# 3ickey/ConsensusML

Hardware: AMD Instinct MI355X
Metric: samples/sec ResNet-50 + Krum at 1/2/4/8 MI355X; agg overhead vs all-reduce (higher is better)
Workload: dtype bf16

## Files before the change

csrc/bindings.cpp:

```cpp
#include <torch/extension.h>
#include <array>
#include <climits>
#include <ATen/hip/HIPContext.h>
#include <c10/core/DeviceGuard.h>

#include "kernels/kernels.h"

namespace {

using at::Tensor;
using c10::optional;

#define CML_CHECK_HIP(expr)                                                               \
  do {                                                                                    \
    hipError_t _e = (expr);                                                               \
    TORCH_CHECK(_e == hipSuccess, "consensusml_amd HIP error: ", hipGetErrorString(_e), " at " \
                #expr " (bindings.cpp:", __LINE__, ")");                                  \
  } while (0)

hipStream_t cur_stream() { return c10::hip::getCurrentHIPStream().stream(); }

int dtype_of(const Tensor& t) {
  if (t.scalar_type() == at::kBFloat16) return cml::DT_BF16;
  TORCH_CHECK(t.scalar_type() == at::kFloat, "expected bf16 or fp32 tensor, got ", t.scalar_type());
// ... 1433 lines not shown
                                            cur_stream()));
  return y;
}

Tensor subsample2(const Tensor& x) {
  check_nhwc(x, "x");
  TORCH_CHECK(x.dim() == 4 && x.size(1) % 8 == 0, "subsample2: 4-D NHWC, C % 8 == 0");
  const int64_t N = x.size(0), C = x.size(1), H = x.size(2), W = x.size(3);
  const c10::DeviceGuard guard(x.device());
  Tensor y = at::empty({N, C, (H + 1) / 2, (W + 1) / 2},
                       x.options().memory_format(at::MemoryFormat::ChannelsLast));
  CML_CHECK_HIP(cml::launch_subsample2(x.data_ptr(), y.data_ptr(), static_cast<int>(N),
                                       static_cast<int>(H), static_cast<int>(W),
                                       static_cast<int>(C), cur_stream()));
  return y;
}

Tensor upsample2_scatter(const Tensor& g_in, int64_t H, int64_t W) {
  Tensor g = g_in.contiguous(at::MemoryFormat::ChannelsLast);
  check_nhwc(g, "g");
  const int64_t N = g.size(0), C = g.size(1);
  TORCH_CHECK(g.dim() == 4 && C % 8 == 0 && g.size(2) == (H + 1) / 2 && g.size(3) == (W + 1) / 2,
              "upsample2_scatter: g [N, C, ceil(H/2), ceil(W/2)], C % 8 == 0");
  const c10::DeviceGuard guard(g.device());
  Tensor dx = at::empty({N, C, H, W}, g.options().memory_format(at::MemoryFormat::ChannelsLast));
  CML_CHECK_HIP(cml::launch_upsample2_scatter(g.data_ptr(), dx.data_ptr(), static_cast<int>(N),
                                              static_cast<int>(H), static_cast<int>(W),
                                              static_cast<int>(C), cur_stream()));
  return dx;
}


Tensor wgrad3x3(const Tensor& dy_in, const Tensor& x, at::ScalarType dtype,
                const optional<Tensor>& zero_in) {
  check_nhwc(x, "x");
  Tensor dy = dy_in.contiguous(at::MemoryFormat::ChannelsLast);
  check_nhwc(dy, "dy");
  TORCH_CHECK(x.dim() == 4 && dy.dim() == 4 && dy.size(0) == x.size(0) && dy.size(2) == x.size(2) &&
                  dy.size(3) == x.size(3), "wgrad3x3: dy / x shapes");
  TORCH_CHECK(dtype == at::kBFloat16 || dtype == at::kFloat, "wgrad3x3: bf16 or fp32 output");
  const int64_t N = x.size(0), Ci = x.size(1), H = x.size(2), W = x.size(3), Co = dy.size(1);
  const c10::DeviceGuard guard(x.device());
  int S = 1, T = 0;
  TORCH_CHECK(cml::wgrad3x3_direct_plan(static_cast<int>(N), static_cast<int>(H),
                                        static_cast<int>(W), static_cast<int>(Co),
                                        static_cast<int>(Ci), &S, &T),
              "wgrad3x3: no plan for this shape (check wgrad3x3_direct_ok first)");
  Tensor zero;
  if (zero_in.has_value() && zero_in->defined()) {
    zero = *zero_in;
    TORCH_CHECK(zero.is_cuda() && zero.device() == x.device() && zero.scalar_type() == at::kBFloat16 &&
                    zero.is_contiguous() && zero.numel() >= 8, "wgrad3x3: zero must be >= 8 bf16");
  } else {
    zero = at::zeros({64}, x.options());
  }
  Tensor part = at::empty({S, Co, 9, Ci}, x.options().dtype(at::kFloat));
  Tensor dw = at::empty({Co, 3, 3, Ci}, x.options().dtype(dtype));
  CML_CHECK_HIP(cml::launch_wgrad3x3_direct(dy.data_ptr(), x.data_ptr(), zero.data_ptr(),
                                            part.data_ptr<float>(), dw.data_ptr(),
                                            dtype == at::kBFloat16, static_cast<int>(N),
                                            static_cast<int>(H), static_cast<int>(W),
                                            static_cast<int>(Co), static_cast<int>(Ci),
                                            cur_stream()));
  return dw.permute({0, 3, 1, 2});
}

bool wgrad3x3s2_ok(int64_t N, int64_t H, int64_t W, int64_t Co, int64_t Ci, int64_t taps) {
  int S = 0;
  return N < (1 << 30) && H < (1 << 15) && W < (1 << 15) && Co < (1 << 20) && Ci < (1 << 20) &&
         (taps == 9 || taps == 1) &&
         cml::wgrad3x3s2_plan(static_cast<int>(N), static_cast<int>(H), static_cast<int>(W),
                              static_cast<int>(Co), static_cast<int>(Ci), &S, static_cast<int>(taps));
}

Tensor wgrad3x3s2(const Tensor& dy_in, const Tensor& x, at::ScalarType dtype,
                  const optional<Tensor>& zero_in, int64_t taps) {
  check_nhwc(x, "x");
  Tensor dy = dy_in.contiguous(at::MemoryFormat::ChannelsLast);
  check_nhwc(dy, "dy");
  TORCH_CHECK(x.dim() == 4 && dy.dim() == 4 && dy.size(0) == x.size(0) &&
                  x.size(2) % 2 == 0 && x.size(3) % 2 == 0 && dy.size(2) * 2 == x.size(2) &&
                  dy.size(3) * 2 == x.size(3), "wgrad3x3s2: dy [N, Co, H/2, W/2], x [N, Ci, H, W]");
  TORCH_CHECK(dtype == at::kBFloat16 || dtype == at::kFloat, "wgrad3x3s2: bf16 or fp32 output");
  const int64_t N = x.size(0), Ci = x.size(1), H = x.size(2), W = x.size(3), Co = dy.size(1);
  TORCH_CHECK(wgrad3x3s2_ok(N, H, W, Co, Ci, taps),
              "wgrad3x3s2: no plan for this shape (check wgrad3x3s2_ok first)");
  const c10::DeviceGuard guard(x.device());
  int S = 1;
  cml::wgrad3x3s2_plan(static_cast<int>(N), static_cast<int>(H), static_cast<int>(W),
                       static_cast<int>(Co), static_cast<int>(Ci), &S, static_cast<int>(taps));
  Tensor zero;
  if (zero_in.has_value() && zero_in->defined()) {
    zero = *zero_in;
    TORCH_CHECK(zero.is_cuda() && zero.device() == x.device() && zero.scalar_type() == at::kBFloat16 &&
                    zero.is_contiguous() && zero.numel() >= 256 && zero.data_ptr() != nullptr &&
                    reinterpret_cast<uintptr_t>(zero.data_ptr()) % 16 == 0,
                "wgrad3x3s2: zero must be >= 256 contiguous 16-B aligned bf16");
// ... 1396 lines not shown
        py::arg("pairs"), py::arg("adapt"), py::arg("trust"), py::arg("wd"), py::arg("eps"),
        py::arg("q"), py::arg("stats"), py::arg("reduced") = py::none());
  m.def("lars_update", &lars_update, "SGD-momentum update with a per-tensor gradient factor",
        py::arg("g"), py::arg("scale"), py::arg("master"), py::arg("s1"), py::arg("q"),
        py::arg("starts"), py::arg("starts_host"), py::arg("pouts"), py::arg("offs"),
        py::arg("lens"), py::arg("lr"), py::arg("momentum"), py::arg("weight_decay"),
        py::arg("nesterov"), py::arg("first"), py::arg("grid_cap") = 0);
  m.def("bn_fwd", &bn_fwd, "fused NHWC BatchNorm(+res)(+ReLU) forward");
  m.def("bn_bwd", &bn_bwd, "fused NHWC BatchNorm(+res)(+ReLU) backward");
  m.def("bn_fwd2", &bn_fwd2, "relu(BN(x1) + BN(x2)) forward (downsample-block tail)");
  m.def("bn_bwd2", &bn_bwd2, "relu(BN(x1) + BN(x2)) backward");
  m.def("bn_relu_maxpool_fwd", &bn_relu_maxpool_fwd, "maxpool(relu(BN(x))) forward (stem)");
  m.def("stem_conv_fwd", &stem_conv_fwd, "ResNet stem 7x7/s2 conv + BN statistics (MFMA)");
  m.def("stem_wgrad", &stem_wgrad, "ResNet stem weight gradient through BN (MFMA, one pass)");
  m.def("maxpool_fwd", &maxpool_fwd, "NHWC bf16 max-pool forward (uint8 argmax)");
  m.def("maxpool_bwd", &maxpool_bwd, "NHWC bf16 max-pool backward (gather)");
  m.def("conv1x1_bn_fwd", &conv1x1_bn_fwd, py::arg("x"), py::arg("w"), py::arg("pro_sc"),
        py::arg("pro_bi"), py::arg("shift"), py::arg("running_mean"), py::arg("running_var"),
        py::arg("stride"), py::arg("stats"), py::arg("eps"), py::arg("momentum"),
        py::arg("gamma") = py::none(), py::arg("beta") = py::none(),
        "fused 1x1 conv forward (MFMA) + BN statistics epilogue + optional BN-ReLU prologue "
        "(+ with gamma / beta that BN's affine sc, bi from the statistics' finalize)");
  m.def("bn_stats", &bn_stats, "training BatchNorm statistics (mean, invstd) only");
  m.def("wgrad1x1", &wgrad1x1, py::arg("dy"), py::arg("x"), py::arg("dtype"),
        py::arg("pro_sc") = py::none(), py::arg("pro_bi") = py::none(),
        py::arg("dz_z") = py::none(), py::arg("dz_mask") = py::none(), py::arg("dz_a") = py::none(),
        py::arg("dz_b") = py::none(), py::arg("dz_c") = py::none(), py::arg("out") = py::none(),
        "weight gradient of a stride-1 1x1 conv (MFMA, split-K)");
  m.def("wgrad3x3s2_ok", &wgrad3x3s2_ok, py::arg("N"), py::arg("H"), py::arg("W"),
        py::arg("Co"), py::arg("Ci"), py::arg("taps") = 9);
  m.def("wgrad3x3s2", &wgrad3x3s2, py::arg("dy"), py::arg("x"), py::arg("dtype"),
        py::arg("zero") = py::none(), py::arg("taps") = 9);
  m.def("wgrad3x3", &wgrad3x3, py::arg("dy"), py::arg("x"), py::arg("dtype"),
        py::arg("zero") = py::none(),
        "weight gradient of a 3x3 stride-1 conv (MFMA, split-K, all nine taps per workgroup: "
        "wgrad3x3.hip) for shapes with wgrad3x3_direct_ok");
  m.def("conv1_bn_bwd_ok", &conv1_bn_bwd_ok, py::arg("M"), py::arg("p"), py::arg("Cin"),
        "whether conv1_bn_bwd takes the shape");
  m.def("conv1_bn_bwd", &conv1_bn_bwd, py::arg("dy"), py::arg("z"), py::arg("gamma"),
        py::arg("beta"), py::arg("mean"), py::arg("invstd"), py::arg("sdz"), py::arg("sdzx"),
        py::arg("x"), py::arg("w"), py::arg("dtype"), py::arg("link") = py::none(),
        py::arg("lmask") = py::none(), py::arg("link_s2") = false, py::arg("want_dz") = false,
        py::arg("splits") = 0,
        "conv1's data and weight gradients with bn1's backward apply formed on chip");
  m.def("conv1x1_link_s2", &conv1x1_link_s2,
        "1x1 data gradient + a stride-2 conv's compact data gradient at the even pixels");
  m.def("subsample2", &subsample2, "x[:, :, ::2, ::2] of an NHWC bf16 tensor, dense NHWC");
  m.def("upsample2_scatter", &upsample2_scatter, py::arg("g"), py::arg("H"), py::arg("W"),
        "full-resolution NHWC tensor with g at the even pixels, zeros elsewhere");
  m.def("wgrad3x3_direct_ok", [](int64_t B, int64_t H, int64_t W, int64_t Co, int64_t Ci) {
    int S, T;
    return cml::wgrad3x3_direct_plan(static_cast<int>(B), static_cast<int>(H), static_cast<int>(W),
                                     static_cast<int>(Co), static_cast<int>(Ci), &S, &T);
  }, "whether wgrad3x3 takes the nine-tap kernel for this shape");
  m.def("conv_gemm_bnsums", &conv_gemm_bnsums, py::arg("x"), py::arg("w"), py::arg("taps"),
        py::arg("zero"), py::arg("z"), py::arg("sc"), py::arg("bi"), py::arg("mean"),
        py::arg("invstd"), py::arg("dgamma_out") = py::none(), py::arg("dbeta_out") = py::none(),
        "stride-1 conv_gemm + the sums of the BN + ReLU backward its output feeds (+ optionally "
        "that BN's parameter gradients)");
  m.def("conv_gemm_s2dgrad", &conv_gemm_s2dgrad, py::arg("dy"), py::arg("wr"), py::arg("zero"),
        py::arg("z") = py::none(), py::arg("sc") = py::none(), py::arg("bi") = py::none(),
        py::arg("mean") = py::none(), py::arg("invstd") = py::none(),
        py::arg("dgamma_out") = py::none(), py::arg("dbeta_out") = py::none(),
        "stride-2 3x3 data gradient as four parity-class implicit GEMMs (+ BN + ReLU backward sums, "
        "+ optionally that BN's parameter gradients)");
  m.def("conv_gemm", &conv_gemm, py::arg("x"), py::arg("w"), py::arg("taps"),
        py::arg("zero") = py::none(), py::arg("stride") = 1,
        "implicit-GEMM NHWC conv (1x1 / 3x3 padding 1, stride 1 or 2), glds staging");
  m.def("conv1x1_bn_stats_only", &conv1x1_bn_stats_only, py::arg("x"), py::arg("w"),
// ... 175 lines not shown
```

csrc/kernels/kernels.h:

```cpp
#pragma once
#include <hip/hip_runtime.h>
#include <stdint.h>

namespace cml {

enum DType : int { DT_BF16 = 0, DT_F32 = 1 };
enum Combine : int { CMB_SORTED = 0, CMB_WEIGHTED = 1 };
enum Opt : int { OPT_NONE = 0, OPT_SGD = 1, OPT_ADAM = 2 };
enum Rule : int {
  RULE_MEAN = 0,
  RULE_KRUM = 1,
  RULE_MULTI_KRUM = 2,
  RULE_GEOMED = 3,
  RULE_CCLIP = 4,
  RULE_BULYAN_SELECT = 5,
  RULE_NNM_ONLY = 6,
};

struct SrcArgs {
  const void* X;
  int64_t ld;
  int n;
  int keep;
  const int* rows;
  const float* w;
  int lo, cnt;
};

struct UpdArgs {
  float* master;
  float* s1;
  float* s2;
  void* param_out;
  float* gout;
  float lr, momentum, weight_decay, beta1, beta2, eps, step_size, inv_sqrt_bc2, gscale;
// ... 253 lines not shown
bool wgrad1x1_direct(int64_t P, int Co, int Ci, bool pro = false, int dmode = 0, bool cs = false);
hipError_t launch_wgrad1x1_ex(const void* dy, const void* x, float* part, void* dw, bool dw_bf16,
                              int64_t P, int Co, int Ci, const float* pro_sc, const float* pro_bi,
                              hipStream_t st, int dmode, const void* dz_z, const uint8_t* dz_mask,
                              const float* dz_a, const float* dz_b, const float* dz_c,
                              float* cs_part, float* cs);
hipError_t launch_wgrad1x1(const void* dy, const void* x, float* part, void* dw, bool dw_bf16,
                           int64_t P, int Co, int Ci, const float* pro_sc, const float* pro_bi,
                           hipStream_t stream, const void* dz_z = nullptr,
                           const uint8_t* dz_mask = nullptr, const float* dz_a = nullptr,
                           const float* dz_b = nullptr, const float* dz_c = nullptr);

void gram1x1_plan(int64_t M, int p, int* splits, int* cps);
hipError_t launch_gram1x1(const void* z, float* part, float* G, int64_t M, int p, const float* sc,
                          const float* bi, float* cs_part, float* cy, hipStream_t st);
bool gram1x1_route(const void* dy, const void* x, int Co, int Ci, const float* pro_sc,
                   const float* pro_bi, int dmode, const float* dz_a, const float* dz_b,
                   bool dw_bf16);

bool conv1_bwd_plan(int64_t M, int p, int Cin, int* splits, int want = 0);
hipError_t launch_conv1_bwd(const void* dy, const void* z, const void* gamma, const void* beta,
                            const float* mean, const float* invstd, const float* sdz,
                            const float* sdzx, const void* x, const void* w, const void* link,
                            const uint8_t* lmask, int link_kind, int Nimg, int H, int W, void* dx,
                            float* part, int splits, void* dw, bool dw_bf16, void* dz_out,
                            int64_t M, int p, int Cin, hipStream_t st);

bool wgrad3x3s2_plan(int N, int H, int W, int Co, int Ci, int* splits, int taps = 9);
hipError_t launch_wgrad3x3s2(const void* dy, const void* x, const void* zero, float* part,
                             void* dw, bool dw_bf16, int N, int H, int W, int Co, int Ci,
                             hipStream_t st, int taps = 9);
hipError_t launch_wgrad_fold(const float* part, int S, int64_t n, void* out, bool out_bf16,
                             hipStream_t st);
bool wgrad3x3_direct_plan(int B, int H, int W, int Co, int Ci, int* splits, int* tci);
hipError_t launch_wgrad3x3_direct(const void* dy, const void* x, const void* zero, float* part,
                                  void* dw, bool dw_bf16, int B, int H, int W, int Co, int Ci,
                                  hipStream_t st);

size_t conv1x1_bn_part_floats(int64_t M, int K, int N, bool pro);
struct BnAffineOut {
  const void* gamma;
  const void* beta;
  float* sc;
  float* bi;
};
hipError_t launch_conv1x1_bn_fwd(const void* x, const void* w, void* y, float* part,
                                 const float* pro_sc, const float* pro_bi, const float* shift,
                                 int64_t M, int K, int N, int stride, int H, int W, float* mean,
                                 float* invstd, float* rmean, float* rvar, float eps,
                                 float momentum, hipStream_t st, const BnAffineOut* aff = nullptr);

size_t conv_gemm_part_floats(int64_t M, int N);
hipError_t launch_conv_gemm_bnsums(const void* x, const void* w, void* y, const void* zero,
                                   int Nimg, int H, int W, int C, int N, int taps, const void* z,
                                   const float* sc, const float* bi, const float* mean,
                                   const float* invstd, float* part, float* sdz, float* sdzx,
                                   hipStream_t st, void* dgamma = nullptr, void* dbeta = nullptr);
hipError_t launch_bnbwd_sums_finalize(const float* part, int R, int BN, int N, const float* invstd,
                                      float* sdz, float* sdzx, hipStream_t st, float* fold,
                                      void* dgamma = nullptr, void* dbeta = nullptr);
size_t conv_gemm_s2dgrad_part_floats(int64_t Mc, int N);
hipError_t launch_conv_gemm_s2dgrad(const void* dy, const void* wr, void* dx, const void* zero,
                                    int Nimg, int Ho, int Wo, int Co, int Ci, const void* z,
                                    const float* sc, const float* bi, const float* mean,
                                    const float* invstd, float* part, float* sdz, float* sdzx,
                                    hipStream_t st, void* dgamma = nullptr, void* dbeta = nullptr);
hipError_t launch_conv3x3_wlayouts(const void* w, int Co, int Ci, int64_t s0, int64_t s1,
                                   int64_t s2, int64_t s3, void* wf, void* wr, hipStream_t st);
struct WlDesc {
  const void* w;
// ... 123 lines not shown
```

csrc/kernels/wgrad3x3.hip:

```cpp
#include <algorithm>
#include <cstdlib>

#include "common.h"
#include "kernels.h"

namespace cml {
namespace {

typedef __bf16 bf16x8_t __attribute__((ext_vector_type(8)));
typedef float f32x16 __attribute__((ext_vector_type(16)));
typedef short s16x4 __attribute__((ext_vector_type(4)));
typedef __attribute__((address_space(3))) s16x4 lds_s16x4;
typedef __attribute__((address_space(3))) void lds_void;
typedef __attribute__((address_space(1))) void g_void;

constexpr int kKP = 112;
constexpr int kKS = kKP / 16;
constexpr int kNW = 12;
constexpr int kRBD = 192;
constexpr int kMaxDyRows = 232;
constexpr int kMaxIX = 3, kMaxID = 4;

__device__ __forceinline__ f32x16 mfma(bf16x8_t a, bf16x8_t b, f32x16 c) {
  return __builtin_amdgcn_mfma_f32_32x32x16_bf16(a, b, c, 0, 0, 0);
}
__device__ __forceinline__ s16x4 ld_tr(const char* p) {
  return __builtin_amdgcn_ds_read_tr16_b64_v4i16((lds_s16x4*)(p));
}
__device__ __forceinline__ bf16x8_t cat(s16x4 a, s16x4 b) {
  return __builtin_bit_cast(bf16x8_t, __builtin_shufflevector(a, b, 0, 1, 2, 3, 4, 5, 6, 7));
}

struct W3Args {
  const uint16_t* dy;
  const uint16_t* x;
  const uint16_t* zero;
  float* part;
  int H, W, Co, Ci;
  int R, G;
  int npx;
  int nch, cps;
  int tiles_ci, tiles;
  int rx, rd;
};

__device__ __forceinline__ int base_row(int k, int W, int HW, int G) {
  const int r = k / W;
  int b = k + 2 * r;
  if (G > 1) b += (k / HW) * (2 * W + 4);
  return b;
}

template <int TCI>
__global__ __launch_bounds__(kNW * 64, 1) void wgrad3x3_kernel(W3Args a) {
  constexpr int NB = TCI / 64;
  constexpr int RBX = TCI * 2 + 64;
  constexpr int SX = RBX / 16, SD = kRBD / 16;
  extern __shared__ __attribute__((aligned(16))) char smem[];
  const int tid = threadIdx.x, lane = tid & 63;
  const int wave = __builtin_amdgcn_readfirstlane(tid >> 6);
  const int dhi = wave >> 2, sub = wave & 3;
  const int cpart = sub & 1, ipart = sub >> 1;
  const int h = lane >> 5, r32 = lane & 31, grp = lane >> 4, gi = lane & 15;
  const int q = gi >> 2, p = gi & 3;
  const int Gb = gridDim.x, b = blockIdx.x, xcd = b & 7, q8 = Gb >> 3, r8 = Gb & 7;
  const int t = (xcd < r8 ? xcd * (q8 + 1) : r8 * (q8 + 1) + (xcd - r8) * q8) + (b >> 3);
  const int tile = t % a.tiles, split = t / a.tiles;
  const int tco = tile / a.tiles_ci, tci = tile - tco * a.tiles_ci;
  const int co0 = tco * 64, ci0 = tci * TCI;
  const int W = a.W, HW = a.H * a.W, W2 = a.W + 2;
  const int PB = (a.G == 1 ? a.R + 2 : a.H + 2) * W2;

  const int nqx = a.rx >> 10, nqd = a.rd >> 10;
  int xo[kMaxIX], dof[kMaxID];
  uint32_t dtop = 0u, dbot = 0u;
#pragma unroll
  for (int i = 0; i < kMaxIX; ++i) {
    const int s = (wave + kNW * i) * 64 + lane, row = s / SX, j = s - row * SX;
    xo[i] = (row < a.npx && j < TCI / 8) ? row * a.Ci + 8 * j : -1;
  }
#pragma unroll
  for (int i = 0; i < kMaxID; ++i) {
    const int s = (wave + kNW * i) * 64 + lane, row = s / SD, j = s - row * SD;
    const int g = row / PB, rem = row - g * PB, pr = rem / W2, pc = rem - pr * W2;
    bool ok = j < 8 && g < a.G && pc >= 1 && pc <= W;
    if (a.G > 1) ok = ok && pr >= 1 && pr <= a.H;
    dof[i] = ok ? ((g * a.H + pr) * W + pc) * a.Co + 8 * j : -1;
    if (a.G == 1 && pr == 0) dtop |= 1u << i;
    if (a.G == 1 && pr == a.R + 1) dbot |= 1u << i;
  }

  auto issue = [&](int c, int buf) {
    int64_t pix0;
    bool topok = true, botok = true;
    if (a.G == 1) {
      const int per = a.H / a.R, img = c / per, h0 = (c - img * per) * a.R;
      pix0 = (static_cast<int64_t>(img) * a.H + h0) * W;
      topok = h0 > 0;
      botok = h0 + a.R < a.H;
    } else {
      pix0 = static_cast<int64_t>(c) * a.G * HW;
    }
    const int64_t xbase = pix0 * a.Ci + ci0;
    const int64_t dbase = (pix0 - W - 1) * a.Co + co0;
    char* xb = smem + buf * (a.rx + a.rd);
    char* db = xb + a.rx;
#pragma unroll
    for (int i = 0; i < kMaxIX; ++i) {
      const int qi = wave + kNW * i;
      if (qi < nqx) {
        const uint16_t* src = xo[i] >= 0 ? a.x + xbase + xo[i] : a.zero;
        __builtin_amdgcn_global_load_lds((g_void*)src, (lds_void*)(xb + qi * 1024), 16, 0, 0);
      }
    }
#pragma unroll
    for (int i = 0; i < kMaxID; ++i) {
      const int qi = wave + kNW * i;
      if (qi < nqd) {
        const bool ok = dof[i] >= 0 && (topok || !((dtop >> i) & 1u)) &&
                        (botok || !((dbot >> i) & 1u));
        const uint16_t* src = ok ? a.dy + dbase + dof[i] : a.zero;
        __builtin_amdgcn_global_load_lds((g_void*)src, (lds_void*)(db + qi * 1024), 16, 0, 0);
      }
    }
  };

  const int chx = 2 * (ipart * 32 * NB + 16 * (grp & 1) + 4 * p);
  const int xa = (8 * h + q) * RBX + chx;
  const int chd = 2 * (cpart * 32 + 16 * (grp & 1) + 4 * p);
  int da0[kKS], da1[kKS];
#pragma unroll
  for (int ks = 0; ks < kKS; ++ks) {
    da0[ks] = base_row(16 * ks + 8 * h + q, W, HW, a.G) * kRBD + chd;
    da1[ks] = base_row(16 * ks + 8 * h + q + 4, W, HW, a.G) * kRBD + chd;
  }
  const int sdh = (2 - dhi) * W2 * kRBD;

  f32x16 acc[3][NB];
#pragma unroll
  for (int i = 0; i < 3; ++i)
#pragma unroll
    for (int j = 0; j < NB; ++j)
#pragma unroll
      for (int k = 0; k < 16; ++k) acc[i][j][k] = 0.f;

  const int c_lo = split * a.cps;
  const int c_hi = min(a.nch, c_lo + a.cps);
  if (c_lo < c_hi) issue(c_lo, 0);
  asm volatile("s_waitcnt vmcnt(0)" ::: "memory");
  __syncthreads();
  for (int c = c_lo; c < c_hi; ++c) {
    const int buf = (c - c_lo) & 1;
    if (c + 1 < c_hi) issue(c + 1, buf ^ 1);
    const char* xb = smem + buf * (a.rx + a.rd);
    const char* db = xb + a.rx + sdh;
#pragma unroll
    for (int ks = 0; ks < kKS; ++ks) {
      bf16x8_t B[NB], A[3];
#pragma unroll
      for (int j = 0; j < NB; ++j) {
        const char* px = xb + xa + 16 * ks * RBX + 64 * j;
        B[j] = cat(ld_tr(px), ld_tr(px + 4 * RBX));
      }
#pragma unroll
      for (int tt = 0; tt < 3; ++tt)
        A[tt] = cat(ld_tr(db + da0[ks] + tt * kRBD), ld_tr(db + da1[ks] + tt * kRBD));
#pragma unroll
      for (int tt = 0; tt < 3; ++tt)
#pragma unroll
        for (int j = 0; j < NB; ++j) acc[tt][j] = mfma(A[tt], B[j], acc[tt][j]);
    }
    asm volatile("s_waitcnt vmcnt(0)" ::: "memory");
    __syncthreads();
  }

  float* pw = a.part + static_cast<int64_t>(split) * a.Co * 9 * a.Ci;
#pragma unroll
  for (int tt = 0; tt < 3; ++tt) {
    const int tap = 3 * dhi + 2 - tt;
#pragma unroll
    for (int j = 0; j < NB; ++j)
#pragma unroll
      for (int k = 0; k < 16; ++k) {
        const int co = co0 + cpart * 32 + (k & 3) + 8 * (k >> 2) + 4 * h;
        const int ci = ci0 + ipart * 32 * NB + 32 * j + r32;
        pw[(static_cast<int64_t>(co) * 9 + tap) * a.Ci + ci] = acc[tt][j][k];
      }
  }
}

int direct_enabled() {
  static const int v = [] {
    const char* e = getenv("CML_WGRAD3X3_DIRECT");
    return e ? atoi(e) : 1;
  }();
  return v;
}

}

bool wgrad3x3_direct_plan(int B, int H, int W, int Co, int Ci, int* splits, int* tci) {
  if (!direct_enabled() || B < 1 || H < 1 || W < 1 || Co % 64 || !(Ci == 64 || Ci % 128 == 0))
    return false;
  int R, G = 1;
  if (H * W <= kKP) {
    R = H;
    for (int g = kKP / (H * W); g >= 1; --g)
      if (B % g == 0) { G = g; break; }
  } else {
    R = 0;
    for (int r = kKP / W; r >= 1; --r)
      if (H % r == 0) { R = r; break; }
    if (R == 0) return false;
  }
  const int k = kKP - 1, HW = H * W;
  const int maxrow = k + 2 * (k / W) + (G > 1 ? (k / HW) * (2 * W + 4) : 0) + 2 * (W + 2) + 2;
  const int PB = (G == 1 ? R + 2 : H + 2) * (W + 2);
  const int dyr = std::max(G * PB, maxrow + 1);
  if (dyr > kMaxDyRows) return false;
  const int T = Ci % 128 == 0 ? 128 : 64;
  const int64_t nch = G == 1 ? static_cast<int64_t>(B) * (H / R) : B / G;
  if (nch >= (1ll << 30)) return false;
  const int tiles = (Co / 64) * (Ci / T);
  int s = (256 + tiles - 1) / tiles;
  s = s < 1 ? 1 : (s > nch ? static_cast<int>(nch) : s);
  const int cps = static_cast<int>((nch + s - 1) / s);
  *splits = static_cast<int>((nch + cps - 1) / cps);
  *tci = T;
  return true;
}

hipError_t launch_wgrad3x3_direct(const void* dy, const void* x, const void* zero, float* part,
                                  void* dw, bool dw_bf16, int B, int H, int W, int Co, int Ci,
                                  hipStream_t st) {
  int S, T;
  if (!wgrad3x3_direct_plan(B, H, W, Co, Ci, &S, &T)) return hipErrorInvalidValue;
  W3Args a{};
  a.dy = reinterpret_cast<const uint16_t*>(dy);
  a.x = reinterpret_cast<const uint16_t*>(x);
  a.zero = reinterpret_cast<const uint16_t*>(zero);
  a.part = part;
  a.H = H;
  a.W = W;
  a.Co = Co;
  a.Ci = Ci;
  const int HW = H * W;
  if (HW <= kKP) {
    a.R = H;
    a.G = 1;
    for (int g = kKP / HW; g >= 1; --g)
      if (B % g == 0) { a.G = g; break; }
  } else {
    a.G = 1;
    for (int r = kKP / W; r >= 1; --r)
      if (H % r == 0) { a.R = r; break; }
  }
  a.npx = a.G * a.R * W;
  a.nch = a.G == 1 ? B * (H / a.R) : B / a.G;
  a.cps = (a.nch + S - 1) / S;
  a.tiles_ci = Ci / T;
  a.tiles = (Co / 64) * a.tiles_ci;
  const int k = kKP - 1;
  const int maxrow = k + 2 * (k / W) + (a.G > 1 ? (k / HW) * (2 * W + 4) : 0) + 2 * (W + 2) + 2;
  const int dyr = std::max(a.G * (a.G == 1 ? a.R + 2 : H + 2) * (W + 2), maxrow + 1);
  a.rx = (kKP * (T * 2 + 64) + 1023) / 1024 * 1024;
  a.rd = (dyr * kRBD + 1023) / 1024 * 1024;
  if ((a.rx >> 10) > kNW * kMaxIX || (a.rd >> 10) > kNW * kMaxID) return hipErrorInvalidValue;
  const size_t lds = 2 * static_cast<size_t>(a.rx + a.rd);
  if (lds > 160 * 1024) return hipErrorInvalidValue;
  const int grid = a.tiles * S;
  auto kern = T == 128 ? &wgrad3x3_kernel<128> : &wgrad3x3_kernel<64>;
  (void)hipFuncSetAttribute(reinterpret_cast<const void*>(kern),
                            hipFuncAttributeMaxDynamicSharedMemorySize, static_cast<int>(lds));
  kern<<<grid, kNW * 64, lds, st>>>(a);
  hipError_t e = hipGetLastError();
  if (e != hipSuccess) return e;
  return launch_wgrad_fold(part, S, 9ll * Co * Ci, dw, dw_bf16, st);
}

}
```

Baseline: 18770.

## Add three-stage ring pipeline with compact swizzled LDS rows to 3x3 wgrad

For 64-channel tiles, the 3x3 weight-gradient kernel now runs a three-buffer ring. Two chunks are prefetched ahead, and a partial vmcnt wait replaces the full drain and barrier after every chunk. LDS rows shrink to 128 bytes with an XOR swizzle to avoid bank conflicts. LDS reads are double-buffered through inline asm with explicit lgkmcnt waits so reads overlap the MFMAs. The change also refactors plan geometry into a shared host/device header, adds a splits override, debug flags and host emulation bindings. The cost is more LDS per workgroup and hand-written waitcnt logic that must match the issue counts.

```diff
diff --git a/csrc/bindings.cpp b/csrc/bindings.cpp
--- a/csrc/bindings.cpp
+++ b/csrc/bindings.cpp
@@ -1489,7 +1489,7 @@
 
 
 Tensor wgrad3x3(const Tensor& dy_in, const Tensor& x, at::ScalarType dtype,
-                const optional<Tensor>& zero_in) {
+                const optional<Tensor>& zero_in, int64_t splits) {
   check_nhwc(x, "x");
   Tensor dy = dy_in.contiguous(at::MemoryFormat::ChannelsLast);
   check_nhwc(dy, "dy");
@@ -1499,9 +1499,10 @@
   const int64_t N = x.size(0), Ci = x.size(1), H = x.size(2), W = x.size(3), Co = dy.size(1);
   const c10::DeviceGuard guard(x.device());
   int S = 1, T = 0;
+  TORCH_CHECK(splits >= 0 && splits < (1 << 30), "wgrad3x3: splits");
   TORCH_CHECK(cml::wgrad3x3_direct_plan(static_cast<int>(N), static_cast<int>(H),
                                         static_cast<int>(W), static_cast<int>(Co),
-                                        static_cast<int>(Ci), &S, &T),
+                                        static_cast<int>(Ci), &S, &T, static_cast<int>(splits)),
               "wgrad3x3: no plan for this shape (check wgrad3x3_direct_ok first)");
   Tensor zero;
   if (zero_in.has_value() && zero_in->defined()) {
@@ -1518,8 +1519,30 @@
                                             dtype == at::kBFloat16, static_cast<int>(N),
                                             static_cast<int>(H), static_cast<int>(W),
                                             static_cast<int>(Co), static_cast<int>(Ci),
-                                            cur_stream()));
+                                            cur_stream(), static_cast<int>(splits)));
   return dw.permute({0, 3, 1, 2});
+}
+
+py::tuple wgrad3x3_geometry_py(int64_t B, int64_t H, int64_t W, int64_t Co, int64_t Ci, int64_t splits) {
+  int g[7];
+  TORCH_CHECK(splits >= 0 && splits < (1 << 30), "wgrad3x3_geometry: splits");
+  TORCH_CHECK(cml::wgrad3x3_geometry(static_cast<int>(B), static_cast<int>(H), static_cast<int>(W),
+                                     static_cast<int>(Co), static_cast<int>(Ci),
+                                     static_cast<int>(splits), g),
+              "wgrad3x3_geometry: no plan for this shape");
+  return py::make_tuple(g[0], g[1], g[2], g[3], g[4], g[5], g[6] != 0);
+}
+
+py::tuple wgrad3x3_plan_emulate_py(int64_t B, int64_t H, int64_t W, int64_t Co, int64_t Ci,
+                                int64_t chunk) {
+  std::vector<int64_t> xs, ds;
+  std::vector<int> kr;
+  TORCH_CHECK(cml::wgrad3x3_plan_emulate(static_cast<int>(B), static_cast<int>(H),
+                                         static_cast<int>(W), static_cast<int>(Co),
+                                         static_cast<int>(Ci), static_cast<int>(chunk), &xs, &ds,
+                                         &kr),
+              "wgrad3x3_plan_emulate: no plan for this shape, or no such chunk");
+  return py::make_tuple(xs, ds, kr);
 }
 
 bool wgrad3x3s2_ok(int64_t N, int64_t H, int64_t W, int64_t Co, int64_t Ci, int64_t taps) {
@@ -2982,9 +3005,15 @@
   m.def("wgrad3x3s2", &wgrad3x3s2, py::arg("dy"), py::arg("x"), py::arg("dtype"),
         py::arg("zero") = py::none(), py::arg("taps") = 9);
   m.def("wgrad3x3", &wgrad3x3, py::arg("dy"), py::arg("x"), py::arg("dtype"),
-        py::arg("zero") = py::none(),
+        py::arg("zero") = py::none(), py::arg("splits") = 0,
         "weight gradient of a 3x3 stride-1 conv (MFMA, split-K, all nine taps per workgroup: "
-        "wgrad3x3.hip) for shapes with wgrad3x3_direct_ok");
+        "wgrad3x3.hip) for shapes with wgrad3x3_direct_ok; splits 0 = the plan's choice");
+  m.def("wgrad3x3_geometry", &wgrad3x3_geometry_py, py::arg("B"), py::arg("H"), py::arg("W"),
+        py::arg("Co"), py::arg("Ci"), py::arg("splits") = 0,
+        "(R, npx, nch, cps, S, stages, stacked) of wgrad3x3's plan");
+  m.def("wgrad3x3_plan_emulate", &wgrad3x3_plan_emulate_py, py::arg("B"), py::arg("H"),
+        py::arg("W"), py::arg("Co"), py::arg("Ci"), py::arg("chunk"),
+        "host emulation of one chunk's DMA plan: (x row sources, dy row sources, k -> padded row)");
   m.def("conv1_bn_bwd_ok", &conv1_bn_bwd_ok, py::arg("M"), py::arg("p"), py::arg("Cin"),
         "whether conv1_bn_bwd takes the shape");
   m.def("conv1_bn_bwd", &conv1_bn_bwd, py::arg("dy"), py::arg("z"), py::arg("gamma"),
diff --git a/csrc/kernels/kernels.h b/csrc/kernels/kernels.h
--- a/csrc/kernels/kernels.h
+++ b/csrc/kernels/kernels.h
@@ -1,6 +1,8 @@
 #pragma once
 #include <hip/hip_runtime.h>
 #include <stdint.h>
+
+#include <vector>
 
 namespace cml {
 
@@ -320,10 +322,13 @@
                              hipStream_t st, int taps = 9);
 hipError_t launch_wgrad_fold(const float* part, int S, int64_t n, void* out, bool out_bf16,
                              hipStream_t st);
-bool wgrad3x3_direct_plan(int B, int H, int W, int Co, int Ci, int* splits, int* tci);
+bool wgrad3x3_direct_plan(int B, int H, int W, int Co, int Ci, int* splits, int* tci, int want = 0);
 hipError_t launch_wgrad3x3_direct(const void* dy, const void* x, const void* zero, float* part,
                                   void* dw, bool dw_bf16, int B, int H, int W, int Co, int Ci,
-                                  hipStream_t st);
+                                  hipStream_t st, int want = 0);
+bool wgrad3x3_geometry(int B, int H, int W, int Co, int Ci, int want, int out[7]);
+bool wgrad3x3_plan_emulate(int B, int H, int W, int Co, int Ci, int chunk, std::vector<int64_t>* xsrc,
+                           std::vector<int64_t>* dysrc, std::vector<int>* krow);
 
 size_t conv1x1_bn_part_floats(int64_t M, int K, int N, bool pro);
 struct BnAffineOut {
diff --git a/csrc/kernels/wgrad3x3.hip b/csrc/kernels/wgrad3x3.hip
--- a/csrc/kernels/wgrad3x3.hip
+++ b/csrc/kernels/wgrad3x3.hip
@@ -3,9 +3,13 @@
 
 #include "common.h"
 #include "kernels.h"
+#include "wgrad3x3_plan.h"
 
 namespace cml {
 namespace {
+
+using w3::kKP;
+using w3::kMaxDyRows;
 
 typedef __bf16 bf16x8_t __attribute__((ext_vector_type(8)));
 typedef float f32x16 __attribute__((ext_vector_type(16)));
@@ -14,11 +18,8 @@
 typedef __attribute__((address_space(3))) void lds_void;
 typedef __attribute__((address_space(1))) void g_void;
 
-constexpr int kKP = 112;
 constexpr int kKS = kKP / 16;
 constexpr int kNW = 12;
-constexpr int kRBD = 192;
-constexpr int kMaxDyRows = 232;
 constexpr int kMaxIX = 3, kMaxID = 4;
 
 __device__ __forceinline__ f32x16 mfma(bf16x8_t a, bf16x8_t b, f32x16 c) {
@@ -27,8 +28,25 @@
 __device__ __forceinline__ s16x4 ld_tr(const char* p) {
   return __builtin_amdgcn_ds_read_tr16_b64_v4i16((lds_s16x4*)(p));
 }
+__device__ __forceinline__ s16x4 ld_tr_asm(int addr) {
+  s16x4 v;
+  asm volatile("ds_read_b64_tr_b16 %0, %1" : "=v"(v) : "v"(addr) : "memory");
+  return v;
+}
 __device__ __forceinline__ bf16x8_t cat(s16x4 a, s16x4 b) {
   return __builtin_bit_cast(bf16x8_t, __builtin_shufflevector(a, b, 0, 1, 2, 3, 4, 5, 6, 7));
+}
+__device__ __forceinline__ void wait_vm(int n) {
+  switch (n) {
+    case 1: asm volatile("s_waitcnt vmcnt(1)" ::: "memory"); break;
+    case 2: asm volatile("s_waitcnt vmcnt(2)" ::: "memory"); break;
+    case 3: asm volatile("s_waitcnt vmcnt(3)" ::: "memory"); break;
+    case 4: asm volatile("s_waitcnt vmcnt(4)" ::: "memory"); break;
+    case 5: asm volatile("s_waitcnt vmcnt(5)" ::: "memory"); break;
+    case 6: asm volatile("s_waitcnt vmcnt(6)" ::: "memory"); break;
+    case 7: asm volatile("s_waitcnt vmcnt(7)" ::: "memory"); break;
+    default: asm volatile("s_waitcnt vmcnt(0)" ::: "memory"); break;
+  }
 }
 
 struct W3Args {
@@ -36,27 +54,24 @@
   const uint16_t* x;
   const uint16_t* zero;
   float* part;
-  int H, W, Co, Ci;
-  int R, G;
-  int npx;
-  int nch, cps;
+  w3::Geo g;
+  int Co, Ci;
+  int cps;
   int tiles_ci, tiles;
   int rx, rd;
+  int dbg;
 };
 
-__device__ __forceinline__ int base_row(int k, int W, int HW, int G) {
-  const int r = k / W;
-  int b = k + 2 * r;
-  if (G > 1) b += (k / HW) * (2 * W + 4);
-  return b;
-}
-
-template <int TCI>
-__global__ __launch_bounds__(kNW * 64, 1) void wgrad3x3_kernel(W3Args a) {
+template <int TCI, bool RING>
+__device__ __forceinline__ void wgrad3x3_body(const W3Args& a) {
+  constexpr bool ASMRD = RING;
+  static_assert(!RING || TCI == 64, "compact rows: 64 channels = one 128-B row");
   constexpr int NB = TCI / 64;
-  constexpr int RBX = TCI * 2 + 64;
-  constexpr int SX = RBX / 16, SD = kRBD / 16;
+  constexpr int RBX = RING ? TCI * 2 : TCI * 2 + 64;
+  constexpr int RBD = RING ? 128 : 192;
+  constexpr int SX = RBX / 16, SD = RBD / 16;
   extern __shared__ __attribute__((aligned(16))) char smem[];
+  const int smem0 = static_cast<int>(reinterpret_cast<uintptr_t>((lds_void*)smem));
   const int tid = threadIdx.x, lane = tid & 63;
   const int wave = __builtin_amdgcn_readfirstlane(tid >> 6);
   const int dhi = wave >> 2, sub = wave & 3;
@@ -68,8 +83,7 @@
   const int tile = t % a.tiles, split = t / a.tiles;
   const int tco = tile / a.tiles_ci, tci = tile - tco * a.tiles_ci;
   const int co0 = tco * 64, ci0 = tci * TCI;
-  const int W = a.W, HW = a.H * a.W, W2 = a.W + 2;
-  const int PB = (a.G == 1 ? a.R + 2 : a.H + 2) * W2;
+  const int W = a.g.W, HW = a.g.H * a.g.W, W2 = a.g.W + 2;
 
   const int nqx = a.rx >> 10, nqd = a.rd >> 10;
   int xo[kMaxIX], dof[kMaxID];
@@ -77,33 +91,26 @@
 #pragma unroll
   for (int i = 0; i < kMaxIX; ++i) {
     const int s = (wave + kNW * i) * 64 + lane, row = s / SX, j = s - row * SX;
-    xo[i] = (row < a.npx && j < TCI / 8) ? row * a.Ci + 8 * j : -1;
+    const int px = w3::x_row_src(a.g, row);
+    xo[i] = (px >= 0 && j < TCI / 8) ? px * a.Ci + 8 * (RING ? w3::swz_slot(row, j) : j) : -1;
   }
 #pragma unroll
   for (int i = 0; i < kMaxID; ++i) {
     const int s = (wave + kNW * i) * 64 + lane, row = s / SD, j = s - row * SD;
-    const int g = row / PB, rem = row - g * PB, pr = rem / W2, pc = rem - pr * W2;
-    bool ok = j < 8 && g < a.G && pc >= 1 && pc <= W;
-    if (a.G > 1) ok = ok && pr >= 1 && pr <= a.H;
-    dof[i] = ok ? ((g * a.H + pr) * W + pc) * a.Co + 8 * j : -1;
-    if (a.G == 1 && pr == 0) dtop |= 1u << i;
-    if (a.G == 1 && pr == a.R + 1) dbot |= 1u << i;
-  }
-
-  auto issue = [&](int c, int buf) {
-    int64_t pix0;
-    bool topok = true, botok = true;
-    if (a.G == 1) {
-      const int per = a.H / a.R, img = c / per, h0 = (c - img * per) * a.R;
-      pix0 = (static_cast<int64_t>(img) * a.H + h0) * W;
-      topok = h0 > 0;
-      botok = h0 + a.R < a.H;
-    } else {
-      pix0 = static_cast<int64_t>(c) * a.G * HW;
-    }
+    bool top, bot;
+    const int px = w3::dy_row_src(a.g, row, &top, &bot);
+    dof[i] = (px >= 0 && j < 8) ? px * a.Co + 8 * (RING ? w3::swz_slot(row, j) : j) : -1;
+    if (top) dtop |= 1u << i;
+    if (bot) dbot |= 1u << i;
+  }
+
+  const int stg = a.rx + a.rd;
+  auto issue = [&](int c, int off) {
+    bool topok, botok;
+    const int64_t pix0 = w3::chunk_origin(a.g, c, &topok, &botok);
     const int64_t xbase = pix0 * a.Ci + ci0;
     const int64_t dbase = (pix0 - W - 1) * a.Co + co0;
-    char* xb = smem + buf * (a.rx + a.rd);
+    char* xb = smem + off;
     char* db = xb + a.rx;
 #pragma unroll
     for (int i = 0; i < kMaxIX; ++i) {
@@ -126,15 +133,25 @@
   };
 
   const int chx = 2 * (ipart * 32 * NB + 16 * (grp & 1) + 4 * p);
-  const int xa = (8 * h + q) * RBX + chx;
+  const int xa = (8 * h + q) * RBX + (RING ? w3::swz_col(q, chx) : chx);
   const int chd = 2 * (cpart * 32 + 16 * (grp & 1) + 4 * p);
+  const int sdh = (2 - dhi) * W2;
   int da0[kKS], da1[kKS];
 #pragma unroll
   for (int ks = 0; ks < kKS; ++ks) {
-    da0[ks] = base_row(16 * ks + 8 * h + q, W, HW, a.G) * kRBD + chd;
-    da1[ks] = base_row(16 * ks + 8 * h + q + 4, W, HW, a.G) * kRBD + chd;
-  }
-  const int sdh = (2 - dhi) * W2 * kRBD;
+    const int r0 = w3::base_row(16 * ks + 8 * h + q, W, HW, a.g.G) + sdh;
+    const int r1 = w3::base_row(16 * ks + 8 * h + q + 4, W, HW, a.g.G) + sdh;
+    da0[ks] = RING ? r0 : r0 * RBD + chd;
+    da1[ks] = RING ? r1 : r1 * RBD + chd;
+  }
+  auto dy_off = [&](int d, int tt) {
+    if constexpr (RING) {
+      const int r = d + tt;
+      return r * RBD + w3::swz_col(r, chd);
+    } else {
+      return d + tt * RBD;
+    }
+  };
 
   f32x16 acc[3][NB];
 #pragma unroll
@@ -144,34 +161,88 @@
 #pragma unroll
       for (int k = 0; k < 16; ++k) acc[i][j][k] = 0.f;
 
+  auto multiply = [&](int off) {
+    const char* xb = smem + off;
+    const char* db = xb + a.rx;
+    const int xi = smem0 + off, di = xi + a.rx;
+    auto mul = [&](const bf16x8_t (&A)[3], const bf16x8_t (&B)[NB]) {
+#pragma unroll
+      for (int tt = 0; tt < 3; ++tt)
+#pragma unroll
+        for (int j = 0; j < NB; ++j) acc[tt][j] = mfma(A[tt], B[j], acc[tt][j]);
+    };
+    if constexpr (ASMRD) {
+      bf16x8_t A[2][3], B[2][NB];
+      auto rd = [&](int ks, int s) {
+#pragma unroll
+        for (int j = 0; j < NB; ++j) {
+          const int px = xi + xa + 16 * ks * RBX + 64 * j;
+          B[s][j] = cat(ld_tr_asm(px), ld_tr_asm(px + 4 * RBX));
+        }
+#pragma unroll
+        for (int tt = 0; tt < 3; ++tt)
+          A[s][tt] = cat(ld_tr_asm(di + dy_off(da0[ks], tt)), ld_tr_asm(di + dy_off(da1[ks], tt)));
+      };
+      rd(0, 0);
+#pragma unroll
+      for (int ks = 0; ks < kKS; ++ks) {
+        if (ks + 1 < kKS) {
+          rd(ks + 1, (ks + 1) & 1);
+          static_assert(2 * NB + 6 == 8, "reads per k-step: the count below");
+          asm volatile("s_waitcnt lgkmcnt(8)" ::: "memory");
+        } else {
+          asm volatile("s_waitcnt lgkmcnt(0)" ::: "memory");
+        }
+        __builtin_amdgcn_sched_barrier(0);
+        mul(A[ks & 1], B[ks & 1]);
+        __builtin_amdgcn_sched_barrier(0);
+      }
+    } else {
+#pragma unroll
+      for (int ks = 0; ks < kKS; ++ks) {
+        bf16x8_t B[NB], A[3];
+#pragma unroll
+        for (int j = 0; j < NB; ++j) {
+          const int px = xa + 16 * ks * RBX + 64 * j;
+          B[j] = cat(ld_tr(xb + px), ld_tr(xb + px + 4 * RBX));
+        }
+#pragma unroll
+        for (int tt = 0; tt < 3; ++tt)
+          A[tt] = cat(ld_tr(db + dy_off(da0[ks], tt)), ld_tr(db + dy_off(da1[ks], tt)));
+        mul(A, B);
+      }
+    }
+  };
+
   const int c_lo = split * a.cps;
-  const int c_hi = min(a.nch, c_lo + a.cps);
-  if (c_lo < c_hi) issue(c_lo, 0);
-  asm volatile("s_waitcnt vmcnt(0)" ::: "memory");
-  __syncthreads();
-  for (int c = c_lo; c < c_hi; ++c) {
-    const int buf = (c - c_lo) & 1;
-    if (c + 1 < c_hi) issue(c + 1, buf ^ 1);
-    const char* xb = smem + buf * (a.rx + a.rd);
-    const char* db = xb + a.rx + sdh;
-#pragma unroll
-    for (int ks = 0; ks < kKS; ++ks) {
-      bf16x8_t B[NB], A[3];
-#pragma unroll
-      for (int j = 0; j < NB; ++j) {
-        const char* px = xb + xa + 16 * ks * RBX + 64 * j;
-        B[j] = cat(ld_tr(px), ld_tr(px + 4 * RBX));
-      }
-#pragma unroll
-      for (int tt = 0; tt < 3; ++tt)
-        A[tt] = cat(ld_tr(db + da0[ks] + tt * kRBD), ld_tr(db + da1[ks] + tt * kRBD));
-#pragma unroll
-      for (int tt = 0; tt < 3; ++tt)
-#pragma unroll
-        for (int j = 0; j < NB; ++j) acc[tt][j] = mfma(A[tt], B[j], acc[tt][j]);
-    }
+  const int c_hi = min(a.g.nch, c_lo + a.cps);
+  const bool domul = !(a.dbg & 1), dodma = !(a.dbg & 2);
+  if constexpr (RING) {
+    const int nvm = (nqx > wave ? (nqx - wave - 1) / kNW + 1 : 0) +
+                    (nqd > wave ? (nqd - wave - 1) / kNW + 1 : 0);
+    const int n = c_hi - c_lo;
+    if (n > 0) issue(c_lo, 0);
+    if (n > 1 && dodma) issue(c_lo + 1, stg);
+    int cur = 0, nxt2 = 2 * stg;
+    for (int i = 0; i < n; ++i) {
+      wait_vm(i + 1 < n ? nvm : 0);
+      asm volatile("s_waitcnt lgkmcnt(0)\n\ts_barrier" ::: "memory");
+      if (i + 2 < n && dodma) issue(c_lo + i + 2, nxt2);
+      if (domul) multiply(dodma ? cur : 0);
+      nxt2 = cur;
+      cur = cur + stg == 3 * stg ? 0 : cur + stg;
+    }
+  } else {
+    if (c_lo < c_hi) issue(c_lo, 0);
     asm volatile("s_waitcnt vmcnt(0)" ::: "memory");
     __syncthreads();
+    for (int c = c_lo; c < c_hi; ++c) {
+      const int buf = (c - c_lo) & 1;
+      if (c + 1 < c_hi && dodma) issue(c + 1, (buf ^ 1) * stg);
+      if (domul) multiply(dodma ? buf * stg : 0);
+      asm volatile("s_waitcnt vmcnt(0)" ::: "memory");
+      __syncthreads();
+    }
   }
 
   float* pw = a.part + static_cast<int64_t>(split) * a.Co * 9 * a.Ci;
@@ -189,93 +260,145 @@
   }
 }
 
+template <int TCI>
+__global__ __launch_bounds__(kNW * 64, 1) void wgrad3x3_kernel(W3Args a) {
+  wgrad3x3_body<TCI, false>(a);
+}
+
+template <int TCI>
+__global__ __launch_bounds__(kNW * 64, 1) void wgrad3x3_ring_kernel(W3Args a) {
+  wgrad3x3_body<TCI, true>(a);
+}
+
+int env_int(const char* name, int dflt) {
+  const char* e = getenv(name);
+  return e ? atoi(e) : dflt;
+}
 int direct_enabled() {
-  static const int v = [] {
-    const char* e = getenv("CML_WGRAD3X3_DIRECT");
-    return e ? atoi(e) : 1;
-  }();
+  static const int v = env_int("CML_WGRAD3X3_DIRECT", 1);
   return v;
 }
-
-}
-
-bool wgrad3x3_direct_plan(int B, int H, int W, int Co, int Ci, int* splits, int* tci) {
+int version() {
+  static const int v = env_int("CML_WGRAD3X3_V", 1);
+  return v;
+}
+
+struct Plan {
+  W3Args a;
+  int S, T, stages;
+  size_t lds;
+};
+
+bool make_plan(int B, int H, int W, int Co, int Ci, int want, Plan* p) {
   if (!direct_enabled() || B < 1 || H < 1 || W < 1 || Co % 64 || !(Ci == 64 || Ci % 128 == 0))
     return false;
-  int R, G = 1;
+  w3::Geo& g = p->a.g;
+  g.H = H;
+  g.W = W;
+  g.G = 1;
   if (H * W <= kKP) {
-    R = H;
-    for (int g = kKP / (H * W); g >= 1; --g)
-      if (B % g == 0) { G = g; break; }
+    g.R = H;
+    for (int k = kKP / (H * W); k >= 1; --k)
+      if (B % k == 0) { g.G = k; break; }
   } else {
-    R = 0;
+    g.R = 0;
     for (int r = kKP / W; r >= 1; --r)
-      if (H % r == 0) { R = r; break; }
-    if (R == 0) return false;
-  }
-  const int k = kKP - 1, HW = H * W;
-  const int maxrow = k + 2 * (k / W) + (G > 1 ? (k / HW) * (2 * W + 4) : 0) + 2 * (W + 2) + 2;
-  const int PB = (G == 1 ? R + 2 : H + 2) * (W + 2);
-  const int dyr = std::max(G * PB, maxrow + 1);
-  if (dyr > kMaxDyRows) return false;
+      if (H % r == 0) { g.R = r; break; }
+    if (g.R == 0) return false;
+  }
+  g.npx = g.G * g.R * W;
+  g.dyr = std::max(g.G * w3::block_rows(g), w3::max_read_row(H, W, g.G) + 1);
+  if (g.dyr > kMaxDyRows) return false;
   const int T = Ci % 128 == 0 ? 128 : 64;
-  const int64_t nch = G == 1 ? static_cast<int64_t>(B) * (H / R) : B / G;
+  const int64_t nch = g.G == 1 ? static_cast<int64_t>(B) * (H / g.R) : B / g.G;
   if (nch >= (1ll << 30)) return false;
+  g.nch = static_cast<int>(nch);
   const int tiles = (Co / 64) * (Ci / T);
-  int s = (256 + tiles - 1) / tiles;
+  int s = want > 0 ? want : (256 + tiles - 1) / tiles;
   s = s < 1 ? 1 : (s > nch ? static_cast<int>(nch) : s);
-  const int cps = static_cast<int>((nch + s - 1) / s);
-  *splits = static_cast<int>((nch + cps - 1) / cps);
-  *tci = T;
+  p->a.cps = static_cast<int>((nch + s - 1) / s);
+  p->S = static_cast<int>((nch + p->a.cps - 1) / p->a.cps);
+  p->T = T;
+  p->a.Co = Co;
+  p->a.Ci = Ci;
+  p->a.tiles_ci = Ci / T;
+  p->a.tiles = tiles;
+  const bool ring = version() >= 1 && T == 64;
+  p->stages = ring ? 3 : 2;
+  p->a.rx = (kKP * (ring ? T * 2 : T * 2 + 64) + 1023) / 1024 * 1024;
+  p->a.rd = (g.dyr * (ring ? 128 : 192) + 1023) / 1024 * 1024;
+  p->lds = static_cast<size_t>(p->stages) * (p->a.rx + p->a.rd);
+  if ((p->a.rx >> 10) > kNW * kMaxIX || (p->a.rd >> 10) > kNW * kMaxID) return false;
+  return p->lds <= 160 * 1024;
+}
+
+}
+
+bool wgrad3x3_direct_plan(int B, int H, int W, int Co, int Ci, int* splits, int* tci, int want) {
+  Plan p{};
+  if (!make_plan(B, H, W, Co, Ci, want, &p)) return false;
+  *splits = p.S;
+  *tci = p.T;
+  return true;
+}
+
+bool wgrad3x3_geometry(int B, int H, int W, int Co, int Ci, int want, int out[7]) {
+  Plan p{};
+  if (!make_plan(B, H, W, Co, Ci, want, &p)) return false;
+  out[0] = p.a.g.R;
+  out[1] = p.a.g.npx;
+  out[2] = p.a.g.nch;
+  out[3] = p.a.cps;
+  out[4] = p.S;
+  out[5] = p.stages;
+  out[6] = 0;
+  return true;
+}
+
+bool wgrad3x3_plan_emulate(int B, int H, int W, int Co, int Ci, int chunk, std::vector<int64_t>* xsrc,
+                           std::vector<int64_t>* dysrc, std::vector<int>* krow) {
+  Plan p{};
+  if (!make_plan(B, H, W, Co, Ci, 0, &p) || chunk < 0 || chunk >= p.a.g.nch) return false;
+  const w3::Geo& g = p.a.g;
+  bool topok, botok;
+  const int64_t pix0 = w3::chunk_origin(g, chunk, &topok, &botok);
+  xsrc->assign(kKP, -1);
+  for (int row = 0; row < kKP; ++row) {
+    const int px = w3::x_row_src(g, row);
+    if (px >= 0) (*xsrc)[row] = (pix0 + px) * Ci;
+  }
+  dysrc->assign(g.dyr, -1);
+  for (int row = 0; row < g.dyr; ++row) {
+    bool top, bot;
+    const int px = w3::dy_row_src(g, row, &top, &bot);
+    if (px >= 0 && (topok || !top) && (botok || !bot)) (*dysrc)[row] = (pix0 - W - 1 + px) * Co;
+  }
+  krow->resize(kKP);
+  for (int k = 0; k < kKP; ++k) (*krow)[k] = w3::base_row(k, W, H * W, g.G) + W + 3;
   return true;
 }
 
 hipError_t launch_wgrad3x3_direct(const void* dy, const void* x, const void* zero, float* part,
                                   void* dw, bool dw_bf16, int B, int H, int W, int Co, int Ci,
-                                  hipStream_t st) {
-  int S, T;
-  if (!wgrad3x3_direct_plan(B, H, W, Co, Ci, &S, &T)) return hipErrorInvalidValue;
-  W3Args a{};
+                                  hipStream_t st, int want) {
+  Plan p{};
+  if (!make_plan(B, H, W, Co, Ci, want, &p)) return hipErrorInvalidValue;
+  W3Args& a = p.a;
   a.dy = reinterpret_cast<const uint16_t*>(dy);
   a.x = reinterpret_cast<const uint16_t*>(x);
   a.zero = reinterpret_cast<const uint16_t*>(zero);
   a.part = part;
-  a.H = H;
-  a.W = W;
-  a.Co = Co;
-  a.Ci = Ci;
-  const int HW = H * W;
-  if (HW <= kKP) {
-    a.R = H;
-    a.G = 1;
-    for (int g = kKP / HW; g >= 1; --g)
-      if (B % g == 0) { a.G = g; break; }
-  } else {
-    a.G = 1;
-    for (int r = kKP / W; r >= 1; --r)
-      if (H % r == 0) { a.R = r; break; }
-  }
-  a.npx = a.G * a.R * W;
-  a.nch = a.G == 1 ? B * (H / a.R) : B / a.G;
-  a.cps = (a.nch + S - 1) / S;
-  a.tiles_ci = Ci / T;
-  a.tiles = (Co / 64) * a.tiles_ci;
-  const int k = kKP - 1;
-  const int maxrow = k + 2 * (k / W) + (a.G > 1 ? (k / HW) * (2 * W + 4) : 0) + 2 * (W + 2) + 2;
-  const int dyr = std::max(a.G * (a.G == 1 ? a.R + 2 : H + 2) * (W + 2), maxrow + 1);
-  a.rx = (kKP * (T * 2 + 64) + 1023) / 1024 * 1024;
-  a.rd = (dyr * kRBD + 1023) / 1024 * 1024;
-  if ((a.rx >> 10) > kNW * kMaxIX || (a.rd >> 10) > kNW * kMaxID) return hipErrorInvalidValue;
-  const size_t lds = 2 * static_cast<size_t>(a.rx + a.rd);
-  if (lds > 160 * 1024) return hipErrorInvalidValue;
-  const int grid = a.tiles * S;
-  auto kern = T == 128 ? &wgrad3x3_kernel<128> : &wgrad3x3_kernel<64>;
+  static const int dbg = env_int("CML_WGRAD3X3_DBG", 0);
+  a.dbg = dbg;
+  const int grid = a.tiles * p.S;
+  auto kern = p.stages == 3 ? &wgrad3x3_ring_kernel<64>
+                            : (p.T == 128 ? &wgrad3x3_kernel<128> : &wgrad3x3_kernel<64>);
   (void)hipFuncSetAttribute(reinterpret_cast<const void*>(kern),
-                            hipFuncAttributeMaxDynamicSharedMemorySize, static_cast<int>(lds));
-  kern<<<grid, kNW * 64, lds, st>>>(a);
+                            hipFuncAttributeMaxDynamicSharedMemorySize, static_cast<int>(p.lds));
+  kern<<<grid, kNW * 64, p.lds, st>>>(a);
   hipError_t e = hipGetLastError();
   if (e != hipSuccess) return e;
-  return launch_wgrad_fold(part, S, 9ll * Co * Ci, dw, dw_bf16, st);
-}
-
-}
+  return launch_wgrad_fold(part, p.S, 9ll * Co * Ci, dw, dw_bf16, st);
+}
+
+}
diff --git a/csrc/kernels/wgrad3x3_plan.h b/csrc/kernels/wgrad3x3_plan.h
--- /dev/null
+++ b/csrc/kernels/wgrad3x3_plan.h
@@ -0,0 +1,66 @@
+#pragma once
+
+#include <cstdint>
+
+#if defined(__HIPCC__) || defined(__CUDACC__)
+#define CML_W3_HD __host__ __device__ __forceinline__
+#else
+#define CML_W3_HD inline
+#endif
+
+namespace cml {
+namespace w3 {
+
+constexpr int kKP = 112;
+constexpr int kMaxDyRows = 232;
+
+struct Geo {
+  int H, W;
+  int R, G;
+  int npx;
+  int nch;
+  int dyr;
+};
+
+CML_W3_HD int base_row(int k, int W, int HW, int G) {
+  const int r = k / W;
+  int b = k + 2 * r;
+  if (G > 1) b += (k / HW) * (2 * W + 4);
+  return b;
+}
+
+CML_W3_HD int block_rows(const Geo& g) { return (g.G == 1 ? g.R + 2 : g.H + 2) * (g.W + 2); }
+
+CML_W3_HD int max_read_row(int H, int W, int G) {
+  return base_row(kKP - 1, W, H * W, G) + 2 * (W + 2) + 2;
+}
+
+CML_W3_HD int64_t chunk_origin(const Geo& g, int c, bool* topok, bool* botok) {
+  if (g.G == 1) {
+    const int per = g.H / g.R, img = c / per, h0 = (c - img * per) * g.R;
+    *topok = h0 > 0;
+    *botok = h0 + g.R < g.H;
+    return (static_cast<int64_t>(img) * g.H + h0) * g.W;
+  }
+  *topok = true;
+  *botok = true;
+  return static_cast<int64_t>(c) * g.G * g.H * g.W;
+}
+
+CML_W3_HD int x_row_src(const Geo& g, int row) { return row < g.npx ? row : -1; }
+
+CML_W3_HD int dy_row_src(const Geo& g, int row, bool* top, bool* bot) {
+  const int W2 = g.W + 2, PB = block_rows(g);
+  const int b = row / PB, rem = row - b * PB, pr = rem / W2, pc = rem - pr * W2;
+  *top = g.G == 1 && pr == 0;
+  *bot = g.G == 1 && pr == g.R + 1;
+  bool ok = b < g.G && pc >= 1 && pc <= g.W;
+  if (g.G > 1) ok = ok && pr >= 1 && pr <= g.H;
+  return ok ? (b * g.H + pr) * g.W + pc : -1;
+}
+
+CML_W3_HD int swz_slot(int row, int j) { return j ^ ((row & 2) << 1); }
+CML_W3_HD int swz_col(int row, int c) { return c ^ ((row & 2) << 5); }
+
+}
+}
```

Result: no change. 18810, median of 4 (+0.2%).
